# PearCoding/PearRay

Hardware: AMD Instinct MI355X
Metric: Msamples/s (higher is better)
Workload: dtype f32; 1 GPU; C4: Cornell box + 999968-triangle soup (1000000 triangles), 1920x1080, `direct` integrator (NEE+MIS+RR, depth 64), sobol 1024-spp schedule, hero wavelengths (spd CMIS), 307 iterations timed; parallelism=tiles1, collective=none (one rank)

## Files before the change

pearray_amd/csrc/device/render.h:

```cpp
#pragma once
#include "pr_device.h"

namespace prd {
constexpr int N_DEVICE_COUNTERS = PRGPU_STAT_COUNT + 32;

struct TraceWorkspace {
	uint32_t* queue_head = nullptr;
	uint2* spill		 = nullptr;
	uint32_t max_blocks	 = 0;
	int refill_below	 = 44;
	uint32_t* bl_list	 = nullptr;
	uint32_t* bl_word	 = nullptr;
	uint32_t* slot_unit	 = nullptr;
	size_t bl_entries	 = 0;
};
size_t trace_workspace_spill_entries(uint32_t max_blocks);
uint32_t trace_stack_capacity();

void launch_raygen(const DevScene& sc, const PathState& ps, uint32_t slot_base, uint32_t n_slots, uint32_t iter, unsigned long long* gstats, hipStream_t st);
void launch_trace_closest(const DevScene& sc, const PathState& ps, const uint32_t* active, uint32_t slot_base, uint32_t n_active, bool count,
						  const TraceWorkspace& ws, uint32_t* shade_counters, unsigned long long* gstats, hipStream_t st);
void launch_shade(const DevScene& sc, const PathState& ps, const uint32_t* active, uint32_t slot_base, uint32_t n_active, uint32_t* next_active,
				  uint32_t* counters, uint32_t* dead_list, uint32_t* queue_head_closest, uint32_t* queue_head_shadow, unsigned long long* gstats,
				  hipStream_t st);
void launch_regen(const DevScene& sc, const PathState& ps, const uint32_t* dead, uint32_t n_dead, uint32_t iter_end, uint32_t* next_active,
				  uint32_t* counters, unsigned long long* gstats, hipStream_t st);
void launch_trace_shadow(const DevScene& sc, const PathState& ps, uint32_t n_items, bool count, const TraceWorkspace& ws, unsigned long long* gstats,
						 hipStream_t st);
struct PersistentGeometry {
	uint32_t n_blocks, slots_per_block;
};
PersistentGeometry persistent_geometry(uint32_t n_owned, uint32_t max_blocks, uint32_t max_slots_per_block);
uint32_t persistent_slot_padding();
uint32_t slot_array_padding();
uint32_t persistent_block_threads();
int shade_ticks_counter();
struct PersistentTuning {
	uint32_t slots	  = 384;
	int shade_min	  = 64;
	int shade_partial = 16;
	int fin_batch	  = 16;
	int occupancy	  = 3;
	int shader_wave	  = -1;
	bool resident	  = true;
};
void launch_path_persistent(const DevScene& sc, const PathState& ps, const uint32_t* owned, uint32_t n_owned, uint32_t iter_begin, uint32_t iter_end,
							bool count, const TraceWorkspace& ws, const PersistentTuning& tune, int shader_waves , uint32_t* next_pixel, uint32_t* error,
							unsigned long long* gstats, hipStream_t st);
struct PathVariant {
	int id;
	uint32_t features;
};
constexpr uint32_t FEAT_NO_LPE = FEAT_ALL & ~(FEAT_LPE | FEAT_QUADRICS | FEAT_DISKS | FEAT_IMAGES | FEAT_MIX_MATERIALS | FEAT_EXPR | FEAT_SCALAR_NODES), FEAT_NO_ROUGH = FEAT_NO_LPE & ~FEAT_ROUGH_MATERIALS;
constexpr PathVariant PATH_VARIANTS[] = { { 1, 0u }, { 2, FEAT_DELTA_MATERIALS }, { 3, FEAT_NO_ROUGH }, { 4, FEAT_NO_LPE }, { 5, FEAT_ALL } };
constexpr int N_PATH_VARIANTS		  = int(sizeof(PATH_VARIANTS) / sizeof(PATH_VARIANTS[0]));
constexpr int path_variant(uint32_t features)
{
	for (int i = 0; i < N_PATH_VARIANTS - 1; ++i)
		if ((features & ~PATH_VARIANTS[i].features) == 0u)
			return i;
	return N_PATH_VARIANTS - 1;
}
constexpr int path_variant_row(int id)
{
	int i = 0;
	while (i < N_PATH_VARIANTS && PATH_VARIANTS[i].id != id)
		++i;
	return i;
}
constexpr bool path_variants_nested()
{
	for (int i = 0; i + 1 < N_PATH_VARIANTS; ++i)
		if ((PATH_VARIANTS[i].features & ~PATH_VARIANTS[i + 1].features) != 0u)
			return false;
	return true;
}
static_assert(PATH_VARIANTS[N_PATH_VARIANTS - 1].features == FEAT_ALL, "the last variant must cover every scene");
constexpr bool expr_rides_with_images()
{
	for (int i = 0; i < N_PATH_VARIANTS; ++i)
		if (((PATH_VARIANTS[i].features & FEAT_IMAGES) != 0u) != ((PATH_VARIANTS[i].features & FEAT_EXPR) != 0u))
			return false;
	return true;
}
static_assert(expr_rides_with_images(), "FEAT_EXPR and FEAT_IMAGES must sit in the same rows: the closures' _uv forms serve both");
static_assert(path_variants_nested(), "each variant's mask must be contained in the next one's: then the first covering row is the smallest covering one");
// ... 79 lines not shown
```

pearray_amd/csrc/device/render.hip:

```cpp
#define PR_WAVEFRONT 1
#define PR_THROUGHPUT 2
#define PR_LATENCY 3
#if !defined(PR_UNIT) || (PR_UNIT != PR_WAVEFRONT && PR_UNIT != PR_THROUGHPUT && PR_UNIT != PR_LATENCY)
#error "compile with -DPR_UNIT=PR_WAVEFRONT, PR_THROUGHPUT or PR_LATENCY (see the Makefile)"
#endif
#include "render.h"

#include <algorithm>
#include <array>
#include <utility>
#if PR_UNIT == PR_WAVEFRONT
#include <hipcub/hipcub.hpp>
#endif

namespace prd {

__device__ __forceinline__ unsigned long long lane_ballot(bool p) { return __builtin_amdgcn_ballot_w64(p); }
__device__ __forceinline__ bool lane_in(unsigned long long m) { return __builtin_amdgcn_inverse_ballot_w64(m); }
__device__ __forceinline__ int wave_popc(unsigned long long m)
{
	int n = __builtin_popcountll(m);
	asm volatile("" : "+s"(n));
	return n;
}

struct Hit {
	float t, u, v;
	uint32_t tri;
};

enum { CNT_NODES_CLOSEST = PRGPU_STAT_COUNT, CNT_TRIS_CLOSEST, CNT_NODES_ANY, CNT_TRIS_ANY, CNT_WAVE_ITERS_CLOSEST, CNT_WAVE_ITERS_ANY, CNT_SHADE_BATCHES, CNT_SHADE_LANES, CNT_SHADE_TICKS, CNT_IDLE_TICKS, CNT_TOTAL_TICKS, CNT_LEAF_TICKS, CNT_INNER_TICKS, CNT_TOTAL_CYCLES, CNT_REFILL_TICKS, CNT_FIN_TICKS, CNT_CAMERA_TICKS, CNT_VERTEX_TICKS,
	   CNT_CLS_TICKS0, CNT_CLS_BATCHES0 = CNT_CLS_TICKS0 + 4, CNT_CLS_LANES0 = CNT_CLS_BATCHES0 + 4,
	   CNT_SINGLES_CLOSEST = CNT_CLS_LANES0 + 4, CNT_SINGLES_ANY };

#ifndef PR_PEEK
#define PR_PEEK 0
#endif
#ifndef PR_PL_VARIANTS
#define PR_PL_VARIANTS 31
#endif
#ifndef PR_PP_BLOCK
#define PR_PP_BLOCK 256
#endif
constexpr int PP_BLOCK		= PR_PP_BLOCK;
constexpr int TRAV_BLOCK	= PR_UNIT != PR_WAVEFRONT ? PP_BLOCK : 256;
constexpr int STACK_LDS		= 16;
constexpr int STACK_SPILL	= 64;

struct Stack {
	uint2* lds;
	uint2* spill;
	uint32_t spill_stride;
	int sp, base;
	__device__ __forceinline__ void reset() { sp = base = 0; }
	__device__ __forceinline__ void reserve(int k)
	{
		while (sp - base + k > STACK_LDS) {
			if (base < STACK_SPILL)
				spill[(uint32_t)base * spill_stride] = lds[(base & (STACK_LDS - 1)) * TRAV_BLOCK];
			++base;
		}
	}
	__device__ __forceinline__ void push_if(bool valid, uint32_t ref, uint32_t key)
	{
		lds[(sp & (STACK_LDS - 1)) * TRAV_BLOCK] = make_uint2(ref, key);
		sp += valid ? 1 : 0;
	}
	__device__ __forceinline__ uint2 peek() const { return lds[((sp - 1) & (STACK_LDS - 1)) * TRAV_BLOCK]; }
	__device__ __forceinline__ uint2 pop_peeked(uint2 top)
	{
		--sp;
		if (__builtin_expect(sp < base, 0)) {
			base = sp;
			top	 = make_uint2(REC_EMPTY, 0x7F800000u);
			if (sp < STACK_SPILL)
				top = spill[(uint32_t)sp * spill_stride];
		}
		return top;
	}
	__device__ __forceinline__ uint2 pop()
	{
		--sp;
		uint2 e = lds[(sp & (STACK_LDS - 1)) * TRAV_BLOCK];
		if (__builtin_expect(sp < base, 0)) {
			base = sp;
			e	 = make_uint2(REC_EMPTY, 0x7F800000u);
// ... 2235 lines not shown
		}
	};
	trace_persistent<true, COUNT>(sc, n, queue_head, spill, refill_below, load, store, gstats);
}

__global__ void __launch_bounds__(256) k_resolve(DevScene sc, PathState ps, uint32_t iter)
{
	const uint32_t W = sc.cfg.width, H = sc.cfg.height;
	const uint32_t p = blockIdx.x * blockDim.x + threadIdx.x;
	if (p >= W * H)
		return;
	float acc[3];
	if (sc.single_tap) {
		acc[0] = ps.iter_xyz[3 * p];
		acc[1] = ps.iter_xyz[3 * p + 1];
		acc[2] = ps.iter_xyz[3 * p + 2];
	} else {
		const int r = (int)sc.cfg.filter_radius, dd = 2 * r + 1;
		const int x = (int)(p % W), y = (int)(p / W);
		acc[0] = acc[1] = acc[2] = 0.0f;
		for (int sy = y - r; sy <= y + r; ++sy) {
			if (sy < 0 || sy >= (int)H)
				continue;
			for (int sx = x - r; sx <= x + r; ++sx) {
				if (sx < 0 || sx >= (int)W)
					continue;
				const float fw = sc.filter[(y - sy + r) * dd + (x - sx + r)];
				if (fw > PR_EPS) {
					const uint32_t q = (uint32_t)sy * W + (uint32_t)sx;
					acc[0] += fw * ps.iter_xyz[3 * q];
					acc[1] += fw * ps.iter_xyz[3 * q + 1];
					acc[2] += fw * ps.iter_xyz[3 * q + 2];
				}
			}
		}
	}
	fold_iteration(ps, p, iter, acc);
}


#endif
#ifndef PR_PP_SLOTS_MAX
#define PR_PP_SLOTS_MAX (PP_BLOCK == 768 ? 1536 : 512)
#endif
#ifndef PR_FIN_PRIO
#define PR_FIN_PRIO 2
#endif
#ifndef PR_REFILL_PRIO
#define PR_REFILL_PRIO 2
#endif
#ifndef PR_SHADE_PRIO
#define PR_SHADE_PRIO 3
#endif
constexpr int PP_SLOTS_MAX		= PR_PP_SLOTS_MAX;
constexpr uint32_t WL_LDS		= 448;
constexpr uint32_t PP_EMPTY		= 0xFFFFFFFFu;
constexpr uint32_t PP_ANY		= 0x80000000u;
constexpr uint32_t PP_DEAD		= 0x100u;
constexpr uint32_t PP_VISIBLE	= 0x200u;
constexpr uint32_t PP_CLS_SHIFT	= 12u;
constexpr uint32_t PP_SHADOW	= 0x400u;
constexpr unsigned long long PP_IDLE_LIMIT_TICKS = 30ull * 100000000ull;

template <int NQ>
struct PPShared {
	uint2 stack[STACK_LDS * TRAV_BLOCK];
	uint32_t q_ray[2 * PP_SLOTS_MAX];
	uint32_t q_shade[NQ + 1][PP_SLOTS_MAX];
	uint32_t pending[PP_SLOTS_MAX];
	uint32_t ray_head, ray_tail, shade_head[NQ + 1], shade_tail[NQ + 1];
	float wl_cdf[WL_LDS];
	uint16_t wl_guide[CDF_GUIDE_BUCKETS + 2];
	uint32_t n_list, unit_next, exhausted, n_frozen;
	uint32_t live;
	uint32_t error;
	BlockStats bs;
};

__device__ __forceinline__ uint32_t lds_load(const uint32_t* p) { return __hip_atomic_load(p, __ATOMIC_RELAXED, __HIP_MEMORY_SCOPE_WORKGROUP); }
__device__ __forceinline__ uint32_t wave_bcast0(uint32_t v) { return (uint32_t)__builtin_amdgcn_readfirstlane((int)v); }

__device__ __forceinline__ void ring_push(uint32_t* q, uint32_t cap_mask, uint32_t* tail, bool pred, uint32_t value)
{
	const unsigned long long mask = __ballot(pred);
	if (mask == 0ull)
		return;
	const uint32_t lane = threadIdx.x & 63u;
	uint32_t base		= 0;
	const int leader	= __ffsll((long long)mask) - 1;
	if ((int)lane == leader)
		base = __hip_atomic_fetch_add(tail, (uint32_t)__popcll(mask), __ATOMIC_RELAXED, __HIP_MEMORY_SCOPE_WORKGROUP);
	base = __shfl(base, leader, 64);
	if (pred)
		__hip_atomic_store(&q[(base + __popcll(mask & ((1ull << lane) - 1ull))) & cap_mask], value, __ATOMIC_RELEASE, __HIP_MEMORY_SCOPE_WORKGROUP);
}
__device__ __forceinline__ uint32_t ring_claim(uint32_t* head, const uint32_t* tail, uint32_t want, uint32_t& first)
{
	uint32_t n = 0, h = 0;
	if ((threadIdx.x & 63u) == 0) {
		h				 = lds_load(head);
		const uint32_t t = lds_load(tail);
		n				 = min(want, t - h);
		if (n) {
			uint32_t expect = h;
			if (!__hip_atomic_compare_exchange_strong(head, &expect, h + n, __ATOMIC_RELAXED, __ATOMIC_RELAXED, __HIP_MEMORY_SCOPE_WORKGROUP))
				n = 0;
		}
	}
	first = wave_bcast0(h);
	return wave_bcast0(n);
}
__device__ __forceinline__ uint32_t ring_take(uint32_t* q, uint32_t cap_mask, uint32_t pos)
{
	uint32_t* e = &q[pos & cap_mask];
	uint32_t v;
	while ((v = __hip_atomic_load(e, __ATOMIC_ACQUIRE, __HIP_MEMORY_SCOPE_WORKGROUP)) == PP_EMPTY)
		__builtin_amdgcn_s_sleep(1);
	__hip_atomic_store(e, PP_EMPTY, __ATOMIC_RELAXED, __HIP_MEMORY_SCOPE_WORKGROUP);
	return v;
}


template <uint32_t FEATS>
__device__ __forceinline__ void apply_deferred_nee(const PathState& ps, uint32_t slot, uint32_t pw)
{
	if (pw & PP_SHADOW) {
		const float4 x		 = ps.st[slot].sh_xyz;
		const uint32_t fbs	 = __float_as_uint(x.w);
		const uint32_t pixel = ps.pixel[slot];
		if (pw & PP_VISIBLE) {
// ... 2 lines not shown
		} else if ((fbs >> 8) & 0xFFu) {
			ps.feedback[pixel] |= (fbs >> 8) & 0xFFu;
		}
	}
}

template <uint32_t FEATS>
__device__ __forceinline__ void fold_ended_sample(const PathState& ps, uint32_t slot, uint32_t pixel, uint32_t iter)
{
	if (ps.cost)
		ps.cost[pixel] += (ps.st[slot].flags & 0xFFu) + 1u;
	if (!ps.plane_stride) {
		const float v[3] = { ps.iter_xyz[3 * pixel], ps.iter_xyz[3 * pixel + 1], ps.iter_xyz[3 * pixel + 2] };
		fold_iteration(ps, pixel, iter, v, (FEATS & FEAT_LPE) != 0u);
	}
}


struct PersistentArgs {
	const uint32_t* owned;
	uint32_t n_owned;
	uint32_t* next_pixel;
	uint32_t* error;
	uint32_t slots_per_block;
	uint32_t iter_begin, iter_end;
	uint2* spill;
	int refill_below;
	uint32_t shade_min;
	uint32_t shade_partial;
	uint32_t shader_wave;
	int fin_batch;
	uint32_t direct_map;
	uint32_t resident;
	uint32_t bl_cap;
	uint32_t* bl_list;
	uint32_t* bl_word;
	uint32_t* slot_unit;
	unsigned long long* gstats;
};
constexpr uint32_t PP_SHADE_HELP = 128u;
constexpr uint32_t BL_UNWRITTEN = 0xFFFFFFFEu, BL_HOLE = 0xFFFFFFFFu;

template <bool COUNT, uint32_t FEATS, int WIDE>
__device__ __forceinline__ void path_persistent(const DevScene& sc, const PathState& ps, const PersistentArgs& a)
{
	constexpr int NQ = (FEATS & FEAT_ROUGH_MATERIALS) ? 2 : 1;
	constexpr int QR = NQ;
	constexpr uint32_t FEATS_PLAIN = FEATS & ~FEAT_ROUGH_MATERIALS;
	__shared__ PPShared<NQ> sh;
	constexpr uint32_t RAY_MASK = 2 * PP_SLOTS_MAX - 1, SHADE_MASK = PP_SLOTS_MAX - 1;
	const uint32_t lane	 = threadIdx.x & 63u;
	const uint32_t block_slots = a.slots_per_block;
	const uint32_t slot0	   = blockIdx.x * block_slots;
	for (uint32_t i = threadIdx.x; i < 2 * PP_SLOTS_MAX; i += TRAV_BLOCK)
		sh.q_ray[i] = PP_EMPTY;
	for (uint32_t i = threadIdx.x; i < PP_SLOTS_MAX; i += TRAV_BLOCK) {
		sh.q_shade[QR][i] = i < block_slots ? i : PP_EMPTY;
		for (int q = 0; q < NQ; ++q)
			sh.q_shade[q][i] = PP_EMPTY;
		sh.pending[i] = 0;
		if (i < block_slots)
			ps.pixel[slot0 + i] = INVALID;
	}
	if (threadIdx.x == 0) {
		sh.ray_head = sh.ray_tail = 0;
		for (int q = 0; q < NQ; ++q)
			sh.shade_head[q] = sh.shade_tail[q] = 0;
		sh.shade_head[QR] = 0;
		sh.shade_tail[QR] = block_slots;
		sh.live					  = block_slots;
		sh.error				  = 0;
		sh.n_list = sh.unit_next = sh.exhausted = sh.n_frozen = 0;
	}
	uint32_t* const bl_list = a.bl_list + size_t(blockIdx.x) * a.bl_cap;
	uint32_t* const bl_word = a.bl_word + size_t(blockIdx.x) * a.bl_cap;
	if (a.resident)
		for (uint32_t i = threadIdx.x; i < a.bl_cap; i += TRAV_BLOCK) {
			bl_list[i] = BL_UNWRITTEN;
			bl_word[i] = 0u;
		}
	const bool wl_in_lds = sc.wl_cdf_size >= 2u && sc.wl_cdf_size <= WL_LDS && sc.cfg.mapper == PRGPU_MAPPER_SPD_CMIS;
	if (wl_in_lds)
		for (uint32_t i = threadIdx.x; i < sc.wl_cdf_size; i += TRAV_BLOCK)
			sh.wl_cdf[i] = sc.wl_cdf[i];
	stats_init(sh.bs);
	__syncthreads();
	if (wl_in_lds) {
		for (uint32_t b = threadIdx.x; b <= CDF_GUIDE_BUCKETS; b += TRAV_BLOCK) {
			const float x = (float)b / (float)CDF_GUIDE_BUCKETS;
			int first = 0, len = (int)sc.wl_cdf_size;
			while (len > 0) {
				const int half = len / 2, middle = first + half;
				if (sh.wl_cdf[middle] <= x) {
					first = middle + 1;
					len -= half + 1;
				} else {
					len = half;
				}
			}
			sh.wl_guide[b] = (uint16_t)first;
		}
		__syncthreads();
	}
	WlTable wlt;
	if (wl_in_lds) {
		wlt.cdf	  = sh.wl_cdf;
		wlt.guide = sh.wl_guide;
	}

	Stack st;
	Trav s;
	trav_attach(s, st, sh.stack, a.spill);
	s.any			  = false;
	bool has_ray	  = false;
	uint32_t my_entry = 0;

	uint32_t spins	  = 0;
	unsigned long long t_idle_since = 0;
	uint32_t cn_c = 0, cl_c = 0, cn_a = 0, cl_a = 0, cs_c = 0, cs_a = 0, witers = 0, wleaf = 0, sbatches = 0, slanes = 0;
	unsigned long long t_shade = 0, t_idle = 0, t_leaf = 0, t_inner = 0, t_refill = 0, t_fin = 0, t_cam = 0, t_vert = 0;
	unsigned long long t_cls[4] = { 0, 0, 0, 0 };
	uint32_t b_cls[4] = { 0, 0, 0, 0 }, l_cls[4] = { 0, 0, 0, 0 };
	const unsigned long long t_start = COUNT ? wall_clock64() : 0ull;
	const unsigned long long c_start = COUNT ? (unsigned long long)clock64() : 0ull;

	const uint32_t shader_idx = 3u;
	const bool shader		  = a.shader_wave != 0u && ((threadIdx.x >> 6) & 3u) + a.shader_wave > shader_idx;
	const uint32_t shade_full = a.shader_wave != 0u ? PP_SHADE_HELP : a.shade_min;
	for (;;) {
		const int n_act	  = __popcll(__ballot(has_ray));
		uint32_t n_shade = wave_bcast0(lds_load(&sh.shade_tail[0]) - lds_load(&sh.shade_head[0]));
		int cls			 = 0;
		for (int q = 1; q < NQ + 1; ++q) {
			const uint32_t nq = wave_bcast0(lds_load(&sh.shade_tail[q]) - lds_load(&sh.shade_head[q]));
			if (nq > n_shade) {
				n_shade = nq;
				cls		= q;
			}
		}
		uint32_t n_queued = wave_bcast0(lds_load(&sh.ray_tail) - lds_load(&sh.ray_head));

		bool shade_now;
		if (shader)
			shade_now = n_shade > 0u;
		else if (a.shader_wave != 0u)
			shade_now = n_shade >= shade_full || (n_queued == 0u && n_shade > 0u && n_act == 0);
		else
			shade_now = n_shade >= a.shade_min || (n_queued == 0u && ((n_shade >= a.shade_partial && n_act < a.refill_below) || (n_shade > 0u && n_act == 0)));
		if (shade_now) {
			uint32_t first;
			const uint32_t n = ring_claim(&sh.shade_head[cls], &sh.shade_tail[cls], 64u, first);
			if (n) {
				spins			  = 0;
#if PR_SHADE_PRIO
				__builtin_amdgcn_s_setprio(PR_SHADE_PRIO);
#endif
				const unsigned long long t0 = COUNT ? wall_clock64() : 0ull;
				if (COUNT && lane == 0) {
					++sbatches;
					slanes += n;
				}
				const bool mine	  = lane < n;
				uint32_t slot_l	  = 0;
				const bool regen_pass = cls == QR;
				const bool regen	  = regen_pass;
				if (mine)
					slot_l = ring_take(sh.q_shade[cls], SHADE_MASK, first + lane);
				const uint32_t slot = slot0 + slot_l;
				if (mine)
					apply_deferred_nee<FEATS>(ps, slot, lds_load(&sh.pending[slot_l]));
				bool alive = false, want_shadow = false;
				float4 sh_o = make_float4(0, 0, 0, 0), sh_d = sh_o, sh_xyz = sh_o;
				const unsigned long long t0v = COUNT ? wall_clock64() : 0ull;
				if (regen_pass) {
				} else if (NQ > 1 && cls == 1) {
					if (mine)
						shade_vertex<FEATS>(sc, ps, slot, sh.bs, alive, want_shadow, sh_o, sh_d, sh_xyz);
				} else {
					if (mine)
						shade_vertex<FEATS_PLAIN>(sc, ps, slot, sh.bs, alive, want_shadow, sh_o, sh_d, sh_xyz);
				}
				if (COUNT)
					t_vert += wall_clock64() - t0v;
				const bool to_regen = !regen_pass && mine && !alive && !want_shadow;
				const bool ended	= mine && regen;
				bool need_pixel	 = false;
				uint32_t iter	 = 0;
				if (ended) {
					const uint32_t pixel = ps.pixel[slot];
					need_pixel			 = true;
					if (pixel != INVALID) {
						iter = ps.iter[slot];
						fold_ended_sample<FEATS>(ps, slot, pixel, iter);
						if (iter + 1 < a.iter_end) {
							if (!a.resident) {
								need_pixel = false;
								iter	   = iter + 1;
							} else {
								const uint32_t old = __hip_atomic_fetch_add(&bl_word[a.slot_unit[slot]], 1u, __ATOMIC_ACQ_REL, __HIP_MEMORY_SCOPE_WORKGROUP);
								if ((old >> 16) >= (old & 0xFFFFu) + 1u) {
									need_pixel = false;
									iter	   = iter + 1;
								}
							}
						}
					}
				}
				bool retired = false;
				if (a.resident) {
					if (wave_bcast0(lds_load(&sh.exhausted)) == 0u) {
						const unsigned long long m = __ballot(need_pixel);
						if (m != 0ull) {
							const uint32_t n	= (uint32_t)__popcll(m);
							const uint32_t rank = (uint32_t)__popcll(m & ((1ull << lane) - 1ull));
							const int leader	= __ffsll((long long)m) - 1;
							uint32_t pos		= 0;
							if ((int)lane == leader)
								pos = __hip_atomic_fetch_add(&sh.n_list, n, __ATOMIC_RELAXED, __HIP_MEMORY_SCOPE_WORKGROUP);
							pos = __shfl(pos, leader, 64);
							const uint32_t n_fit = pos >= a.bl_cap ? 0u : min(n, a.bl_cap - pos);
							uint32_t idx		 = a.n_owned;
							if (n_fit != 0u) {
								__builtin_amdgcn_fence(__ATOMIC_SEQ_CST, "workgroup");
								if ((int)lane == leader)
									idx = atomicAdd(a.next_pixel, n_fit);
								idx = __shfl(idx, leader, 64);
							}
							if ((n_fit < n || idx + n_fit >= a.n_owned) && (int)lane == leader)
								__hip_atomic_store(&sh.exhausted, 1u, __ATOMIC_RELEASE, __HIP_MEMORY_SCOPE_WORKGROUP);
							if (need_pixel && rank < n_fit) {
								const uint32_t i = idx + rank;
								uint32_t entry	 = BL_HOLE;
								if (i < a.n_owned) {
// ... 62 lines not shown
							iter		   = a.iter_begin;
						} else {
							retired = true;
						}
					}
				}
				const unsigned long long t0c = COUNT ? wall_clock64() : 0ull;
				if (ended && !retired) {
					ps.iter[slot] = iter;
					camera_path(sc, ps, slot, iter, sh.bs, (FEATS & FEAT_LPE) != 0u, wlt);
					alive = true;
				}
				if (COUNT)
					t_cam += wall_clock64() - t0c;
				const int n_retired = __popcll(__ballot(retired));
				if (n_retired && lane == 0)
					__hip_atomic_fetch_sub(&sh.live, (uint32_t)n_retired, __ATOMIC_RELAXED, __HIP_MEMORY_SCOPE_WORKGROUP);
				if (mine && !retired) {
					if (want_shadow) {
						ps.st[slot].sh_o	= sh_o;
						ps.st[slot].sh_d	= sh_d;
						ps.st[slot].sh_xyz = sh_xyz;
					}
					__hip_atomic_store(&sh.pending[slot_l], (alive ? 1u : 0u) + (want_shadow ? 1u + PP_SHADOW : 0u) + (alive ? 0u : PP_DEAD), __ATOMIC_RELAXED,
									   __HIP_MEMORY_SCOPE_WORKGROUP);
				}
				ring_push(sh.q_shade[QR], SHADE_MASK, &sh.shade_tail[QR], to_regen, slot_l);
				ring_push(sh.q_ray, RAY_MASK, &sh.ray_tail, want_shadow, slot_l | PP_ANY);
				ring_push(sh.q_ray, RAY_MASK, &sh.ray_tail, alive, slot_l);
				{
					const uint32_t pslot = slot0 + (has_ray ? (my_entry & ~PP_ANY) : 0u);
					const bool pany		 = has_ray && (my_entry & PP_ANY) != 0;
					const float4 ro = pany ? ps.st[pslot].sh_o : ps.st[pslot].ray_o, rd = pany ? ps.st[pslot].sh_d : ps.st[pslot].ray_d;
					s.r	   = ray_prepare(v3(ro.x, ro.y, ro.z), v3(rd.x, rd.y, rd.z), sc.eps_t);
					s.tmin = ro.w + 0.0f;
					s.any  = pany;
				}
#if PR_SHADE_PRIO
				__builtin_amdgcn_s_setprio(0);
#endif
				if (COUNT)
					t_shade += wall_clock64() - t0;
				if (COUNT && lane == 0)
					for (int q = 0; q < NQ + 1; ++q)
						if (q == cls) {
							t_cls[q] += wall_clock64() - t0;
							b_cls[q] += 1u;
							l_cls[q] += n;
						}
			}
			continue;
		}

		const unsigned long long idle = __ballot(!has_ray);
		if (!shader && idle != 0ull && n_queued > 0u) {
#if PR_REFILL_PRIO
			__builtin_amdgcn_s_setprio(PR_REFILL_PRIO);
#endif
			const unsigned long long t0r = COUNT ? wall_clock64() : 0ull;
			uint32_t first;
			const uint32_t n = ring_claim(&sh.ray_head, &sh.ray_tail, (uint32_t)__popcll(idle), first);
			const uint32_t r = __popcll(idle & ((1ull << lane) - 1ull));
			if (!has_ray && r < n) {
				my_entry			= ring_take(sh.q_ray, RAY_MASK, first + r);
				const uint32_t slot = slot0 + (my_entry & ~PP_ANY);
				const bool any		= (my_entry & PP_ANY) != 0;
				const float4 ro = any ? ps.st[slot].sh_o : ps.st[slot].ray_o, rd = any ? ps.st[slot].sh_d : ps.st[slot].ray_d;
				trav_begin(s, st, v3(ro.x, ro.y, ro.z), v3(rd.x, rd.y, rd.z), ro.w, any ? rd.w - 0.001f : rd.w, sc.eps_t);
				s.any	= any;
				has_ray = true;
				if (FEATS & FEAT_QUADRICS)
					trav_quadrics<(NQ > 1)>(sc, s, any);
			}
#if PR_REFILL_PRIO
			__builtin_amdgcn_s_setprio(0);
#endif
			if (COUNT)
				t_refill += wall_clock64() - t0r;
		}
		if (!__any(has_ray)) {
			if (lds_load(&sh.live) == 0u || lds_load(&sh.error) != 0u)
				break;
			const unsigned long long t0 = COUNT ? wall_clock64() : 0ull;
			__builtin_amdgcn_s_sleep(8);
			if (COUNT)
				t_idle += wall_clock64() - t0;
			if (n_shade == 0u && n_queued == 0u) {
				if (spins++ == 0u)
					t_idle_since = wall_clock64();
				else if ((spins & 1023u) == 0u && wall_clock64() - t_idle_since > PP_IDLE_LIMIT_TICKS) {
					if (lane == 0) {
						__hip_atomic_store(&sh.error, 1u, __ATOMIC_RELAXED, __HIP_MEMORY_SCOPE_WORKGROUP);
						atomicExch(a.error, 1u);
					}
					break;
				}
			}
			continue;
		}
		spins = 0;
		unsigned long long m_has  = lane_ballot(has_ray);
		unsigned long long m_wait = m_has & lane_ballot(s.cur == REC_EMPTY);
		for (;;) {
			const unsigned long long m_lb	 = lane_ballot((s.cur & REC_LEAF_BIT) != 0u);
			const unsigned long long m_leaf	 = m_has & m_lb & ~m_wait;
			const unsigned long long m_inner = m_has & ~m_lb;
			const int n_leaf = wave_popc(m_leaf), n_inner = wave_popc(m_inner);
			if (COUNT && lane == 0)
				++witers;
			const bool do_inner = n_inner >= n_leaf;
			const unsigned long long t0s = COUNT ? wall_clock64() : 0ull;
			if (lane_in(do_inner ? m_inner : m_leaf)) {
				const float4* __restrict__ rec = rec_ptr(sc.recs, s.cur);
				const float4 q0 = rec[0], q1 = rec[1], q2 = rec[2];
				const bool wide = WIDE == 2 ? sc.bvh_wide != 0u : WIDE == 1;
				float4 qw		= make_float4(0.0f, 0.0f, 0.0f, 0.0f);
				if (wide && do_inner)
					qw = rec[3];
				const uint2 top_e	   = PR_PEEK ? st.peek() : make_uint2(0u, 0u);
				const uint2* const top = PR_PEEK ? &top_e : nullptr;
				if (do_inner) {
					if (COUNT) {
						cn_c += s.any ? 0 : 1;
						cn_a += s.any ? 1 : 0;
					}
					trav_inner_rec<MODE_MIXED>(s, st, q0, q1, q2, qw, wide, top);
				} else {
					float4 q3 = make_float4(0.0f, 0.0f, 0.0f, 0.0f), q4 = q3, q5 = q3, q6 = q3, q7 = q3;
					if (!(s.cur & REC_SINGLE_BIT)) {
						q3 = rec[3];
						q4 = rec[4];
						q5 = rec[5];
						q6 = rec[6];
						q7 = rec[7];
					}
					if (COUNT) {
						cl_c += s.any ? 0 : 1;
						cl_a += s.any ? 1 : 0;
						if (s.cur & REC_SINGLE_BIT) {
							cs_c += s.any ? 0 : 1;
							cs_a += s.any ? 1 : 0;
						}
					}
					trav_leaf_rec<MODE_MIXED, (FEATS & ANA_ALL), (NQ > 1)>(s, st, q0, q1, q2, q3, q4, q5, q6, q7, top);
				}
			}
			if (COUNT) {
				if (do_inner)
					t_inner += wall_clock64() - t0s;
				else
					t_leaf += wall_clock64() - t0s;
			}
			const unsigned long long m_done = m_has & lane_ballot(s.cur == REC_EMPTY);
			unsigned long long m_fin		= m_done;
			if (a.fin_batch > 1) {
				const int n_done = wave_popc(m_done);
				const int n_run	 = wave_popc(m_has & ~m_done);
				if (n_done < a.fin_batch && n_run >= a.refill_below)
					m_fin = 0ull;
			}
			const unsigned long long t0f = COUNT ? wall_clock64() : 0ull;
			if (m_fin != 0ull) {
#if PR_FIN_PRIO
				__builtin_amdgcn_s_setprio(PR_FIN_PRIO);
#endif
				const bool fin = lane_in(m_fin);
				bool last	   = false;
				uint32_t entry = 0;
				int qcls	   = 0;
				if (fin) {
					const uint32_t slot_l = my_entry & ~PP_ANY;
					const uint32_t slot	  = slot0 + slot_l;
					uint32_t add = 0xFFFFFFFFu;
					if (s.any) {
						if (s.best.tri == INVALID)
							add += PP_VISIBLE;
					} else {
						ps.st[slot].hit = make_float4(s.best.t, s.best.u, s.best.v, __uint_as_float(s.best.tri));
						if (NQ > 1)
							add += (s.cls & 3u) << PP_CLS_SHIFT;
					}
					const uint32_t old = __hip_atomic_fetch_add(&sh.pending[slot_l], add, __ATOMIC_ACQ_REL, __HIP_MEMORY_SCOPE_WORKGROUP);
					last			   = (old & 0xFFu) == 1u;
					entry			   = slot_l;
					if (last && (old & PP_DEAD))
						qcls = QR;
					if (NQ > 1 && last && !(old & PP_DEAD))
						qcls = s.any ? (int)((old >> PP_CLS_SHIFT) & 3u) : (int)(s.cls & 3u);
				}
				m_has &= ~m_fin;
				for (int q = 0; q < NQ + 1; ++q)
					ring_push(sh.q_shade[q], SHADE_MASK, &sh.shade_tail[q], last && qcls == q, entry);
#if PR_FIN_PRIO
				__builtin_amdgcn_s_setprio(0);
#endif
				if (COUNT)
					t_fin += wall_clock64() - t0f;
			}
			m_wait			 = m_done & m_has;
			const int active = wave_popc(m_has);
			if (active == 0)
				break;
			if (active < a.refill_below) {
				uint32_t nsh = lds_load(&sh.shade_tail[0]) - lds_load(&sh.shade_head[0]);
				for (int q = 1; q < NQ + 1; ++q)
					nsh = max(nsh, lds_load(&sh.shade_tail[q]) - lds_load(&sh.shade_head[q]));
				const uint32_t nq = lds_load(&sh.ray_tail) - lds_load(&sh.ray_head);
				if (wave_bcast0((nq > 0u || nsh >= shade_full || (a.shader_wave == 0u && nsh >= a.shade_partial)) ? 1u : 0u))
					break;
			}
		}
		has_ray = lane_in(m_has);
	}
	if (COUNT) {
		if (cn_c)
			atomicAdd(&a.gstats[CNT_NODES_CLOSEST], (unsigned long long)cn_c);
		if (cl_c)
			atomicAdd(&a.gstats[CNT_TRIS_CLOSEST], (unsigned long long)cl_c);
		if (cn_a)
			atomicAdd(&a.gstats[CNT_NODES_ANY], (unsigned long long)cn_a);
		if (cl_a)
			atomicAdd(&a.gstats[CNT_TRIS_ANY], (unsigned long long)cl_a);
		if (cs_c)
			atomicAdd(&a.gstats[CNT_SINGLES_CLOSEST], (unsigned long long)cs_c);
		if (cs_a)
			atomicAdd(&a.gstats[CNT_SINGLES_ANY], (unsigned long long)cs_a);
		if (witers)
			atomicAdd(&a.gstats[CNT_WAVE_ITERS_CLOSEST], (unsigned long long)witers);
		if (wleaf)
			atomicAdd(&a.gstats[CNT_WAVE_ITERS_ANY], (unsigned long long)wleaf);
		if (sbatches) {
			atomicAdd(&a.gstats[CNT_SHADE_BATCHES], (unsigned long long)sbatches);
			atomicAdd(&a.gstats[CNT_SHADE_LANES], (unsigned long long)slanes);
		}
		if (lane == 0) {
			atomicAdd(&a.gstats[CNT_SHADE_TICKS], t_shade);
			atomicAdd(&a.gstats[CNT_IDLE_TICKS], t_idle);
			atomicAdd(&a.gstats[CNT_TOTAL_TICKS], wall_clock64() - t_start);
			atomicAdd(&a.gstats[CNT_LEAF_TICKS], t_leaf);
			atomicAdd(&a.gstats[CNT_INNER_TICKS], t_inner);
			atomicAdd(&a.gstats[CNT_REFILL_TICKS], t_refill);
			atomicAdd(&a.gstats[CNT_FIN_TICKS], t_fin);
			atomicAdd(&a.gstats[CNT_CAMERA_TICKS], t_cam);
			atomicAdd(&a.gstats[CNT_VERTEX_TICKS], t_vert);
			atomicAdd(&a.gstats[CNT_TOTAL_CYCLES], (unsigned long long)clock64() - c_start);
			for (int q = 0; q < NQ + 1; ++q) {
				atomicAdd(&a.gstats[CNT_CLS_TICKS0 + q], t_cls[q]);
				atomicAdd(&a.gstats[CNT_CLS_BATCHES0 + q], (unsigned long long)b_cls[q]);
				atomicAdd(&a.gstats[CNT_CLS_LANES0 + q], (unsigned long long)l_cls[q]);
			}
		}
		if (threadIdx.x == 0)
			a.spill[blockIdx.x * TRAV_BLOCK] = make_uint2((uint32_t)(wall_clock64() - t_start), sh.bs.v[PRGPU_STAT_CAMERA_DEPTH] + sh.bs.v[PRGPU_STAT_BACKGROUND_HITS]);
	}
	stats_flush(sh.bs, a.gstats);
}
template <bool COUNT, uint32_t FEATS>
__global__ void __launch_bounds__(TRAV_BLOCK) __attribute__((amdgpu_waves_per_eu(2, 2))) k_path_persistent(DevScene sc, PathState ps, PersistentArgs a)
{
	path_persistent<COUNT, FEATS, 2>(sc, ps, a);
}
template <bool COUNT, uint32_t FEATS, bool WIDE>
__global__ void __launch_bounds__(TRAV_BLOCK) __attribute__((amdgpu_waves_per_eu(3, 3))) k_path_persistent_occ3(DevScene sc, PathState ps, PersistentArgs a)
{
	path_persistent<COUNT, FEATS, WIDE ? 1 : 0>(sc, ps, a);
}

#include "path_wave.inl"

#if PR_UNIT == PR_WAVEFRONT
struct CameraVertex {
	uint32_t pixel;
	float4 hit4;
	V3 ray_d, P;
	GeomPoint gp;
};
enum { CV_NONE, CV_BACKGROUND, CV_HIT };
__device__ __forceinline__ int camera_vertex(const DevScene& sc, const PathState& ps, uint32_t slot, uint32_t n_slots, BlockStats& bs, CameraVertex& cv)
{
	if (slot >= n_slots || (ps.st[slot].flags & FLAG_NO_RAY))
		return CV_NONE;
	const uint32_t pixel = ps.pixel[slot];
	const float4 hit4	 = ps.st[slot].hit;
	const uint32_t tri	 = __float_as_uint(hit4.w);
	cv.pixel			 = pixel;
	cv.hit4				 = hit4;
	if (tri == INVALID) {
		ps.prim_entity[pixel] = INVALID;
		ps.prim_prim[pixel]	  = INVALID;
		atomicAdd(&bs.v[PRGPU_STAT_BACKGROUND_HITS], 1u);
		return CV_BACKGROUND;
	}
	const float4 ro = ps.st[slot].ray_o, rd = ps.st[slot].ray_d;
	const V3 ray_o = v3(ro.x, ro.y, ro.z), ray_d = v3(rd.x, rd.y, rd.z);
	const V3 P = ray_o + ray_d * hit4.x;
	geometry_point<(FEAT_ALL & ~FEAT_LPE)>(sc, tri, hit4.y, hit4.z, P, cv.gp);
	ps.prim_entity[pixel] = cv.gp.entity;
	ps.prim_prim[pixel]	  = cv.gp.prim;
// ... 438 lines not shown
}
bool ao_counts_folded() { return PR_AO_FOLD != 0; }
void launch_vf_shade(const DevScene& sc, const PathState& ps, const VfState& vf, uint32_t n_slots, uint32_t* queue_head_closest, unsigned long long* gstats, hipStream_t st)
{
	hipLaunchKernelGGL(k_vf_shade, grid_for(n_slots), dim3(256), 0, st, sc, ps, vf, n_slots, queue_head_closest, gstats);
}

#endif

template <int VARIANT, int SUB>
void launch_pp(const DevScene& sc, const PathState& ps, const PersistentArgs& a, dim3 grid, hipStream_t st);
template <int VARIANT, int SUB>
void launch_pl(const DevScene& sc, const PathState& ps, const WaveArgs& a, dim3 grid, hipStream_t st);
#if PR_UNIT != PR_WAVEFRONT
#if !defined(PR_VARIANT) || !defined(PR_SUB)
#error "compile the persistent-kernel units with -DPR_VARIANT=<id of a row of PATH_VARIANTS> -DPR_SUB=<index>"
#endif
static_assert(path_variant_row(PR_VARIANT) < N_PATH_VARIANTS, "PR_VARIANT is not the id of a row of PATH_VARIANTS");
#if PR_UNIT == PR_LATENCY
template <int VARIANT, int SUB>
void launch_pl(const DevScene& sc, const PathState& ps, const WaveArgs& a, dim3 grid, hipStream_t st)
{
	static_assert(SUB == 0 || SUB == 1, "latency units: PR_SUB=0 (plain) or 1 (instrumented)");
	hipLaunchKernelGGL((k_path_latency<SUB != 0, PATH_VARIANTS[path_variant_row(VARIANT)].features>), grid, dim3(TRAV_BLOCK), 0, st, sc, ps, a);
}
template void launch_pl<PR_VARIANT, PR_SUB>(const DevScene&, const PathState&, const WaveArgs&, dim3, hipStream_t);
#else
template <int VARIANT, int SUB>
void launch_pp(const DevScene& sc, const PathState& ps, const PersistentArgs& a, dim3 grid, hipStream_t st)
{
	constexpr PathSub u		 = PATH_SUBS[SUB];
	constexpr uint32_t FEATS = PATH_VARIANTS[path_variant_row(VARIANT)].features;
	const dim3 block(TRAV_BLOCK);
	if constexpr (u.occupancy == 3)
		hipLaunchKernelGGL((k_path_persistent_occ3<u.count, FEATS, u.wide>), grid, block, 0, st, sc, ps, a);
	else
		hipLaunchKernelGGL((k_path_persistent<u.count, FEATS>), grid, block, 0, st, sc, ps, a);
}
template void launch_pp<PR_VARIANT, PR_SUB>(const DevScene&, const PathState&, const PersistentArgs&, dim3, hipStream_t);
#endif
#endif

#if PR_UNIT == PR_WAVEFRONT
PersistentGeometry persistent_geometry(uint32_t n_owned, uint32_t max_blocks, uint32_t max_slots_per_block)
{
	PersistentGeometry g;
	const uint32_t per_block = (n_owned + max_blocks - 1) / std::max(1u, max_blocks);
	const uint32_t cap		 = std::min((uint32_t)PP_SLOTS_MAX, std::max(256u, max_slots_per_block / 64u * 64u));
	g.slots_per_block		 = std::min(cap, std::max(64u, per_block));
	g.n_blocks				 = std::max(1u, std::min(max_blocks, (n_owned + g.slots_per_block - 1) / g.slots_per_block));
	return g;
}
uint32_t persistent_slot_padding() { return PP_SLOTS_MAX; }
uint32_t slot_array_padding() { return std::max<uint32_t>(PP_SLOTS_MAX, (TRAV_BLOCK / 64u) * PW_SLOTS_MAX); }
uint32_t persistent_block_threads() { return PP_BLOCK; }
int shade_ticks_counter() { return CNT_SHADE_TICKS; }

typedef void (*PpLaunchFn)(const DevScene&, const PathState&, const PersistentArgs&, dim3, hipStream_t);
typedef void (*PlLaunchFn)(const DevScene&, const PathState&, const WaveArgs&, dim3, hipStream_t);
template <int... I>
constexpr std::array<PpLaunchFn, sizeof...(I)> pp_launch_table(std::integer_sequence<int, I...>)
{
	return { { launch_pp<PATH_VARIANTS[I / N_PATH_SUBS].id, I % N_PATH_SUBS>... } };
}
constexpr bool pl_variant_built(int row) { return ((PR_PL_VARIANTS >> (PATH_VARIANTS[row].id - 1)) & 1u) != 0u; }
template <int ROW, int SUB>
constexpr PlLaunchFn pl_launcher()
{
	if constexpr (pl_variant_built(ROW))
		return launch_pl<PATH_VARIANTS[ROW].id, SUB>;
	else
		return nullptr;
}
template <int... I>
constexpr std::array<PlLaunchFn, sizeof...(I)> pl_launch_table(std::integer_sequence<int, I...>)
{
	return { { pl_launcher<I / 2, I % 2>()... } };
}

void launch_path_persistent(const DevScene& sc, const PathState& ps, const uint32_t* owned, uint32_t n_owned, uint32_t iter_begin, uint32_t iter_end,
							bool count, const TraceWorkspace& ws, const PersistentTuning& tune, int shader_waves, uint32_t* next_pixel, uint32_t* error,
							unsigned long long* gstats, hipStream_t st)
{
	const uint32_t max_slots_per_block = tune.slots;
	const PersistentGeometry g = persistent_geometry(n_owned, ws.max_blocks, max_slots_per_block);
	const bool all_in_flight   = uint64_t(g.n_blocks) * g.slots_per_block >= n_owned;
	PersistentArgs a;
	a.owned			  = owned;
	a.n_owned		  = n_owned;
	a.next_pixel	  = next_pixel;
	a.error			  = error;
	a.slots_per_block = g.slots_per_block;
	a.iter_begin	  = iter_begin;
	a.iter_end		  = iter_end;
	a.spill			  = ws.spill;
	a.refill_below	  = ws.refill_below;
	a.shade_min		  = (uint32_t)std::min(64, std::max(1, tune.shade_min));
	a.shade_partial	  = (uint32_t)std::min(64, std::max(1, tune.shade_partial));
	a.shader_wave	  = PP_BLOCK == 256 ? (uint32_t)std::min(2, std::max(0, shader_waves)) : (shader_waves ? 1u : 0u);
	a.gstats		  = gstats;
	a.direct_map	  = all_in_flight ? 1u : 0u;
	a.fin_batch		  = std::min(64, std::max(1, tune.fin_batch));
	const bool resident_ok = tune.resident;
	a.bl_cap		  = (uint32_t)std::min<uint64_t>(n_owned, 2ull * ((n_owned + g.n_blocks - 1) / g.n_blocks) + 1024ull);
	a.bl_list		  = ws.bl_list;
	a.bl_word		  = ws.bl_word;
// ... 60 lines not shown
```

pearray_amd/csrc/prgpu_api.hip:

```cpp
#include <hip/hip_runtime.h>
#include <dlfcn.h>

#include <algorithm>
#include <climits>
#include <cmath>
#include <cstdlib>
#include <cstring>
#include <map>
#include <string>
#include <vector>

#include "../../include/prgpu.h"
#include "device/bvh.h"
#include "device/render.h"
#include "host/mix_tree.h"
#include "host/setup.h"
#include "tables/pr_vf_colors.inl"
static_assert(sizeof(PR_VF_COLOR_RGB) / sizeof(PR_VF_COLOR_RGB[0]) == prd::VF_COLOURS, "one row per colour index of device/render.h");

namespace {

thread_local std::string g_error;

int fail(int code, const std::string& msg)
// ... 1456 lines not shown

int prgpu_film_size(prgpu_scene* s, uint32_t* width, uint32_t* height)
{
	if (!s)
		return fail(PRGPU_EINVAL, "null scene");
	if (width)
		*width = s->cfg.width;
	if (height)
		*height = s->cfg.height;
	return PRGPU_OK;
}

int prgpu_trace_counters_get(prgpu_scene* s, prgpu_trace_counters* out)
{
	if (!s || !out)
		return fail(PRGPU_EINVAL, "null argument");
	HIP_TRY(hipSetDevice(s->device));
	HIP_TRY(hipStreamSynchronize(s->stream));
	unsigned long long host[prd::N_DEVICE_COUNTERS];
	HIP_TRY(hipMemcpy(host, s->gstats, sizeof(host), hipMemcpyDeviceToHost));
	out->rays_closest  = s->rays_closest;
	out->rays_any	   = s->rays_any;
	if (s->mode == prgpu_scene::PERSISTENT || s->ao_enabled || s->vf_enabled) {
		out->rays_closest += host[PRGPU_STAT_PRIMARY_RAYS] + host[PRGPU_STAT_BOUNCE_RAYS];
		out->rays_any += host[PRGPU_STAT_SHADOW_RAYS];
	}
	out->nodes_closest = host[PRGPU_STAT_COUNT + 0];
	out->leaves_closest  = host[PRGPU_STAT_COUNT + 1];
	out->nodes_any	   = host[PRGPU_STAT_COUNT + 2];
	out->leaves_any	   = host[PRGPU_STAT_COUNT + 3];
	out->node_bytes	   = sizeof(prd::Rec64);
	out->leaf_bytes	   = 2 * sizeof(prd::Rec64);
	if (s->bvh_leaf == 1) {
		out->leaf_bytes		= sizeof(prd::Rec64);
		out->leaves_closest = 2 * out->leaves_closest - host[PRGPU_STAT_COUNT + 30];
		out->leaves_any		= 2 * out->leaves_any - host[PRGPU_STAT_COUNT + 31];
	}
	out->ray_bytes	   = 32;
	out->hit_bytes	   = 16;
	out->wave_steps_closest = host[PRGPU_STAT_COUNT + 4];
	out->wave_steps_any		= host[PRGPU_STAT_COUNT + 5];
	out->shade_batches		= host[PRGPU_STAT_COUNT + 6];
	out->shade_lanes		= host[PRGPU_STAT_COUNT + 7];
	out->shade_ticks		= host[PRGPU_STAT_COUNT + 8];
	out->idle_ticks			= host[PRGPU_STAT_COUNT + 9];
	out->total_ticks		= host[PRGPU_STAT_COUNT + 10];
	if (read_knobs().debug_counters)
		if (host[PRGPU_STAT_COUNT + 10]) {
			const double T = double(host[PRGPU_STAT_COUNT + 10]);
			fprintf(stderr, "[prgpu] wave time: shading %.1f %%, idle %.1f %%, leaf steps %.1f %%, inner steps %.1f %%, refill %.1f %%, ray ends %.1f %%; of the shading: vertices %.1f %%, camera paths %.1f %%; shader clock %.0f MHz\n",
					100 * host[PRGPU_STAT_COUNT + 8] / T, 100 * host[PRGPU_STAT_COUNT + 9] / T, 100 * host[PRGPU_STAT_COUNT + 11] / T, 100 * host[PRGPU_STAT_COUNT + 12] / T,
					100 * host[PRGPU_STAT_COUNT + 14] / T, 100 * host[PRGPU_STAT_COUNT + 15] / T, 100 * host[PRGPU_STAT_COUNT + 17] / T, 100 * host[PRGPU_STAT_COUNT + 16] / T,
					100.0 * double(host[PRGPU_STAT_COUNT + 13]) / T);
			for (int q = 0; q < 4; ++q)
				if (host[PRGPU_STAT_COUNT + 22 + q])
					fprintf(stderr, "[prgpu]   shade queue %d: %.1f %% of wave time, %.0f passes, fill %.3f, %.2f us per pass\n", q, 100 * host[PRGPU_STAT_COUNT + 18 + q] / T,
							double(host[PRGPU_STAT_COUNT + 22 + q]), double(host[PRGPU_STAT_COUNT + 26 + q]) / (64.0 * double(host[PRGPU_STAT_COUNT + 22 + q])),
							0.01 * double(host[PRGPU_STAT_COUNT + 18 + q]) / double(host[PRGPU_STAT_COUNT + 22 + q]));
		}
	return PRGPU_OK;
}

int prgpu_set_instrumentation(prgpu_scene* s, int enabled)
{
	if (!s)
		return fail(PRGPU_EINVAL, "null scene");
	s->instrument = enabled != 0;
	return PRGPU_OK;
}

int prgpu_set_timing(prgpu_scene* s, int enabled)
{
	if (!s)
		return fail(PRGPU_EINVAL, "null scene");
	HIP_TRY(hipSetDevice(s->device));
	HIP_TRY(hipStreamSynchronize(s->stream));
	s->collect_timing();
	s->timing = enabled != 0;
	return PRGPU_OK;
}

int prgpu_kernel_time_ms(prgpu_scene* s, const char* family, double* total_ms, uint64_t* launches)
{
	if (!s || !family)
		return fail(PRGPU_EINVAL, "null argument");
	HIP_TRY(hipSetDevice(s->device));
	HIP_TRY(hipStreamSynchronize(s->stream));
	s->collect_timing();
	for (int f = 0; f < N_FAMILIES; ++f)
		if (std::strcmp(family, FAMILY_NAMES[f]) == 0) {
			if (total_ms)
				*total_ms = s->family_ms[f];
			if (launches)
				*launches = s->family_launches[f];
			return PRGPU_OK;
		}
	return fail(PRGPU_EINVAL, "unknown kernel family");
}

int prgpu_trace_closest(prgpu_scene* s, uint32_t n, const float* org, const float* dir, const float* tmin, const float* tmax,
						uint32_t* entity, uint32_t* prim, float* u, float* v, float* t)
{
	if (!s || (n && (!org || !dir || !tmin || !tmax)))
		return fail(PRGPU_EINVAL, "null argument");
	if (n == 0)
		return PRGPU_OK;
// ... 679 lines not shown
```

Measured before the change: 224.9 Msamples/s.

## Overlap ray pickup with traversal steps and keep hit records in LDS

Splits the refill of idle lanes into an issue phase (claiming queue entries and loading ray origin and direction from global slot records) and a finish phase (traversal setup) that runs after the next traversal step. This lets the global loads overlap with BVH stepping instead of breaking out of the inner loop whenever rays are queued. Closest-hit results are also kept in a per-block LDS array and passed to shade_vertex, avoiding a global store and reload when the block's slot count fits. The LDS footprint grows, and static_asserts check that three 256-lane blocks still fit per CU. New lane-step counters and a debug print are added.

New measurement: 222.5 Msamples/s. 1.1% lower.

```diff
diff --git a/pearray_amd/csrc/device/render.h b/pearray_amd/csrc/device/render.h
--- a/pearray_amd/csrc/device/render.h
+++ b/pearray_amd/csrc/device/render.h
@@ -2,7 +2,7 @@
 #include "pr_device.h"
 
 namespace prd {
-constexpr int N_DEVICE_COUNTERS = PRGPU_STAT_COUNT + 32;
+constexpr int N_DEVICE_COUNTERS = PRGPU_STAT_COUNT + 36;
 
 struct TraceWorkspace {
 	uint32_t* queue_head = nullptr;
@@ -32,6 +32,7 @@
 };
 PersistentGeometry persistent_geometry(uint32_t n_owned, uint32_t max_blocks, uint32_t max_slots_per_block);
 uint32_t persistent_slot_padding();
+uint32_t persistent_hit_slots(uint32_t features);
 uint32_t slot_array_padding();
 uint32_t persistent_block_threads();
 int shade_ticks_counter();
diff --git a/pearray_amd/csrc/device/render.hip b/pearray_amd/csrc/device/render.hip
--- a/pearray_amd/csrc/device/render.hip
+++ b/pearray_amd/csrc/device/render.hip
@@ -31,7 +31,8 @@
 
 enum { CNT_NODES_CLOSEST = PRGPU_STAT_COUNT, CNT_TRIS_CLOSEST, CNT_NODES_ANY, CNT_TRIS_ANY, CNT_WAVE_ITERS_CLOSEST, CNT_WAVE_ITERS_ANY, CNT_SHADE_BATCHES, CNT_SHADE_LANES, CNT_SHADE_TICKS, CNT_IDLE_TICKS, CNT_TOTAL_TICKS, CNT_LEAF_TICKS, CNT_INNER_TICKS, CNT_TOTAL_CYCLES, CNT_REFILL_TICKS, CNT_FIN_TICKS, CNT_CAMERA_TICKS, CNT_VERTEX_TICKS,
 	   CNT_CLS_TICKS0, CNT_CLS_BATCHES0 = CNT_CLS_TICKS0 + 4, CNT_CLS_LANES0 = CNT_CLS_BATCHES0 + 4,
-	   CNT_SINGLES_CLOSEST = CNT_CLS_LANES0 + 4, CNT_SINGLES_ANY };
+	   CNT_SINGLES_CLOSEST = CNT_CLS_LANES0 + 4, CNT_SINGLES_ANY,
+	   CNT_LANES_STEPPED, CNT_LANES_OTHER, CNT_LANES_WAITING, CNT_LANES_EMPTY, CNT_END };
 
 #ifndef PR_PEEK
 #define PR_PEEK 0
@@ -2373,7 +2374,14 @@
 #ifndef PR_SHADE_PRIO
 #define PR_SHADE_PRIO 3
 #endif
+#ifndef PR_PP_PICKUP
+#define PR_PP_PICKUP 1
+#endif
+#ifndef PR_PP_HIT_LDS
+#define PR_PP_HIT_LDS 1
+#endif
 constexpr int PP_SLOTS_MAX		= PR_PP_SLOTS_MAX;
+constexpr uint32_t pp_hit_slots(int nq) { return PR_PP_HIT_LDS ? (nq > 1 ? uint32_t(PP_SLOTS_MAX) * 3u / 4u : uint32_t(PP_SLOTS_MAX)) : 1u; }
 constexpr uint32_t WL_LDS		= 448;
 constexpr uint32_t PP_EMPTY		= 0xFFFFFFFFu;
 constexpr uint32_t PP_ANY		= 0x80000000u;
@@ -2389,6 +2397,7 @@
 	uint32_t q_ray[2 * PP_SLOTS_MAX];
 	uint32_t q_shade[NQ + 1][PP_SLOTS_MAX];
 	uint32_t pending[PP_SLOTS_MAX];
+	float4 hit[pp_hit_slots(NQ)];
 	uint32_t ray_head, ray_tail, shade_head[NQ + 1], shade_tail[NQ + 1];
 	float wl_cdf[WL_LDS];
 	uint16_t wl_guide[CDF_GUIDE_BUCKETS + 2];
@@ -2397,6 +2406,11 @@
 	uint32_t error;
 	BlockStats bs;
 };
+static_assert(CNT_END == N_DEVICE_COUNTERS, "render.h: N_DEVICE_COUNTERS must hold every counter");
+constexpr size_t LDS_UNIT = 1280, LDS_UNITS_PER_CU = 128;
+static_assert(PP_BLOCK != 256 || 3 * ((sizeof(PPShared<2>) + LDS_UNIT - 1) / LDS_UNIT) <= LDS_UNITS_PER_CU, "three blocks of 256 lanes must fit a CU's LDS");
+static_assert(PP_BLOCK != 256 || 3 * ((sizeof(PPShared<1>) + LDS_UNIT - 1) / LDS_UNIT) <= LDS_UNITS_PER_CU, "three blocks of 256 lanes must fit a CU's LDS");
+static_assert(sizeof(PPShared<2>) <= LDS_UNIT * LDS_UNITS_PER_CU, "a block must fit a CU's LDS");
 
 __device__ __forceinline__ uint32_t lds_load(const uint32_t* p) { return __hip_atomic_load(p, __ATOMIC_RELAXED, __HIP_MEMORY_SCOPE_WORKGROUP); }
 __device__ __forceinline__ uint32_t wave_bcast0(uint32_t v) { return (uint32_t)__builtin_amdgcn_readfirstlane((int)v); }
@@ -2505,6 +2519,7 @@
 	const uint32_t lane	 = threadIdx.x & 63u;
 	const uint32_t block_slots = a.slots_per_block;
 	const uint32_t slot0	   = blockIdx.x * block_slots;
+	const bool hit_lds = PR_PP_HIT_LDS && block_slots <= pp_hit_slots(NQ);
 	for (uint32_t i = threadIdx.x; i < 2 * PP_SLOTS_MAX; i += TRAV_BLOCK)
 		sh.q_ray[i] = PP_EMPTY;
 	for (uint32_t i = threadIdx.x; i < PP_SLOTS_MAX; i += TRAV_BLOCK) {
@@ -2574,11 +2589,12 @@
 	unsigned long long t_shade = 0, t_idle = 0, t_leaf = 0, t_inner = 0, t_refill = 0, t_fin = 0, t_cam = 0, t_vert = 0;
 	unsigned long long t_cls[4] = { 0, 0, 0, 0 };
 	uint32_t b_cls[4] = { 0, 0, 0, 0 }, l_cls[4] = { 0, 0, 0, 0 };
+	unsigned long long ls_step = 0, ls_other = 0, ls_wait = 0, ls_empty = 0;
 	const unsigned long long t_start = COUNT ? wall_clock64() : 0ull;
 	const unsigned long long c_start = COUNT ? (unsigned long long)clock64() : 0ull;
 
 	const uint32_t shader_idx = 3u;
-	const bool shader		  = a.shader_wave != 0u && ((threadIdx.x >> 6) & 3u) + a.shader_wave > shader_idx;
+	const bool shader		  = wave_bcast0((a.shader_wave != 0u && ((threadIdx.x >> 6) & 3u) + a.shader_wave > shader_idx) ? 1u : 0u) != 0u;
 	const uint32_t shade_full = a.shader_wave != 0u ? PP_SHADE_HELP : a.shade_min;
 	for (;;) {
 		const int n_act	  = __popcll(__ballot(has_ray));
@@ -2625,13 +2641,20 @@
 				bool alive = false, want_shadow = false;
 				float4 sh_o = make_float4(0, 0, 0, 0), sh_d = sh_o, sh_xyz = sh_o;
 				const unsigned long long t0v = COUNT ? wall_clock64() : 0ull;
+				float4 hit4 = make_float4(0.0f, 0.0f, 0.0f, 0.0f);
+				if (!regen_pass && mine) {
+					if (hit_lds)
+						hit4 = sh.hit[slot_l];
+					else
+						hit4 = ps.st[slot].hit;
+				}
 				if (regen_pass) {
 				} else if (NQ > 1 && cls == 1) {
 					if (mine)
-						shade_vertex<FEATS>(sc, ps, slot, sh.bs, alive, want_shadow, sh_o, sh_d, sh_xyz);
+						shade_vertex<FEATS>(sc, ps, slot, sh.bs, alive, want_shadow, sh_o, sh_d, sh_xyz, &hit4);
 				} else {
 					if (mine)
-						shade_vertex<FEATS_PLAIN>(sc, ps, slot, sh.bs, alive, want_shadow, sh_o, sh_d, sh_xyz);
+						shade_vertex<FEATS_PLAIN>(sc, ps, slot, sh.bs, alive, want_shadow, sh_o, sh_d, sh_xyz, &hit4);
 				}
 				if (COUNT)
 					t_vert += wall_clock64() - t0v;
@@ -2800,33 +2823,52 @@
 			continue;
 		}
 
+		auto pickup_issue = [&](unsigned long long m_idle) -> unsigned long long {
+			uint32_t first;
+			const uint32_t n = ring_claim(&sh.ray_head, &sh.ray_tail, (uint32_t)wave_popc(m_idle), first);
+			const uint32_t r = __popcll(m_idle & ((1ull << lane) - 1ull));
+			const bool take	 = lane_in(m_idle) && r < n;
+			if (take) {
+				my_entry			= ring_take(sh.q_ray, RAY_MASK, first + r);
+				const uint32_t slot = slot0 + (my_entry & ~PP_ANY);
+				const bool any		= (my_entry & PP_ANY) != 0;
+				const float4 ro = any ? ps.st[slot].sh_o : ps.st[slot].ray_o, rd = any ? ps.st[slot].sh_d : ps.st[slot].ray_d;
+				s.r.o	 = v3(ro.x, ro.y, ro.z);
+				s.r.d	 = v3(rd.x, rd.y, rd.z);
+				s.tmin	 = ro.w;
+				s.best.t = rd.w;
+			}
+			return lane_ballot(take);
+		};
+		auto pickup_finish = [&](unsigned long long m_arriving) {
+			if (lane_in(m_arriving)) {
+				const bool any = (my_entry & PP_ANY) != 0;
+				trav_begin(s, st, s.r.o, s.r.d, s.tmin, any ? s.best.t - 0.001f : s.best.t, sc.eps_t);
+				s.any = any;
+				if (FEATS & FEAT_QUADRICS)
+					trav_quadrics<(NQ > 1)>(sc, s, any);
+			}
+		};
+		unsigned long long m_arr	  = 0ull;
 		const unsigned long long idle = __ballot(!has_ray);
 		if (!shader && idle != 0ull && n_queued > 0u) {
 #if PR_REFILL_PRIO
 			__builtin_amdgcn_s_setprio(PR_REFILL_PRIO);
 #endif
 			const unsigned long long t0r = COUNT ? wall_clock64() : 0ull;
-			uint32_t first;
-			const uint32_t n = ring_claim(&sh.ray_head, &sh.ray_tail, (uint32_t)__popcll(idle), first);
-			const uint32_t r = __popcll(idle & ((1ull << lane) - 1ull));
-			if (!has_ray && r < n) {
-				my_entry			= ring_take(sh.q_ray, RAY_MASK, first + r);
-				const uint32_t slot = slot0 + (my_entry & ~PP_ANY);
-				const bool any		= (my_entry & PP_ANY) != 0;
-				const float4 ro = any ? ps.st[slot].sh_o : ps.st[slot].ray_o, rd = any ? ps.st[slot].sh_d : ps.st[slot].ray_d;
-				trav_begin(s, st, v3(ro.x, ro.y, ro.z), v3(rd.x, rd.y, rd.z), ro.w, any ? rd.w - 0.001f : rd.w, sc.eps_t);
-				s.any	= any;
-				has_ray = true;
-				if (FEATS & FEAT_QUADRICS)
-					trav_quadrics<(NQ > 1)>(sc, s, any);
-			}
+			m_arr						 = pickup_issue(idle);
+#if !PR_PP_PICKUP
+			pickup_finish(m_arr);
+			has_ray = has_ray || lane_in(m_arr);
+			m_arr	= 0ull;
+#endif
 #if PR_REFILL_PRIO
 			__builtin_amdgcn_s_setprio(0);
 #endif
 			if (COUNT)
 				t_refill += wall_clock64() - t0r;
 		}
-		if (!__any(has_ray)) {
+		if (!__any(has_ray) && m_arr == 0ull) {
 			if (lds_load(&sh.live) == 0u || lds_load(&sh.error) != 0u)
 				break;
 			const unsigned long long t0 = COUNT ? wall_clock64() : 0ull;
@@ -2857,6 +2899,12 @@
 			if (COUNT && lane == 0)
 				++witers;
 			const bool do_inner = n_inner >= n_leaf;
+			if (COUNT) {
+				ls_step += (unsigned long long)(do_inner ? n_inner : n_leaf);
+				ls_other += (unsigned long long)(do_inner ? n_leaf : n_inner);
+				ls_wait += (unsigned long long)wave_popc(m_wait);
+				ls_empty += (unsigned long long)(64 - wave_popc(m_has));
+			}
 			const unsigned long long t0s = COUNT ? wall_clock64() : 0ull;
 			if (lane_in(do_inner ? m_inner : m_leaf)) {
 				const float4* __restrict__ rec = rec_ptr(sc.recs, s.cur);
@@ -2899,6 +2947,14 @@
 				else
 					t_leaf += wall_clock64() - t0s;
 			}
+			if (m_arr != 0ull) {
+				const unsigned long long t0r = COUNT ? wall_clock64() : 0ull;
+				pickup_finish(m_arr);
+				m_has |= m_arr;
+				m_arr = 0ull;
+				if (COUNT)
+					t_refill += wall_clock64() - t0r;
+			}
 			const unsigned long long m_done = m_has & lane_ballot(s.cur == REC_EMPTY);
 			unsigned long long m_fin		= m_done;
 			if (a.fin_batch > 1) {
@@ -2924,7 +2980,11 @@
 						if (s.best.tri == INVALID)
 							add += PP_VISIBLE;
 					} else {
-						ps.st[slot].hit = make_float4(s.best.t, s.best.u, s.best.v, __uint_as_float(s.best.tri));
+						const float4 h = make_float4(s.best.t, s.best.u, s.best.v, __uint_as_float(s.best.tri));
+						if (hit_lds)
+							sh.hit[slot_l] = h;
+						else
+							ps.st[slot].hit = h;
 						if (NQ > 1)
 							add += (s.cls & 3u) << PP_CLS_SHIFT;
 					}
@@ -2954,8 +3014,20 @@
 				for (int q = 1; q < NQ + 1; ++q)
 					nsh = max(nsh, lds_load(&sh.shade_tail[q]) - lds_load(&sh.shade_head[q]));
 				const uint32_t nq = lds_load(&sh.ray_tail) - lds_load(&sh.ray_head);
+#if PR_PP_PICKUP
+				const uint32_t todo = wave_bcast0((nsh >= shade_full || (nq == 0u && a.shader_wave == 0u && nsh >= a.shade_partial)) ? 2u : (nq > 0u ? 1u : 0u));
+				if (todo == 2u)
+					break;
+				if (todo == 1u) {
+					const unsigned long long t0r = COUNT ? wall_clock64() : 0ull;
+					m_arr						 = pickup_issue(~m_has);
+					if (COUNT)
+						t_refill += wall_clock64() - t0r;
+				}
+#else
 				if (wave_bcast0((nq > 0u || nsh >= shade_full || (a.shader_wave == 0u && nsh >= a.shade_partial)) ? 1u : 0u))
 					break;
+#endif
 			}
 		}
 		has_ray = lane_in(m_has);
@@ -2992,6 +3064,10 @@
 			atomicAdd(&a.gstats[CNT_CAMERA_TICKS], t_cam);
 			atomicAdd(&a.gstats[CNT_VERTEX_TICKS], t_vert);
 			atomicAdd(&a.gstats[CNT_TOTAL_CYCLES], (unsigned long long)clock64() - c_start);
+			atomicAdd(&a.gstats[CNT_LANES_STEPPED], ls_step);
+			atomicAdd(&a.gstats[CNT_LANES_OTHER], ls_other);
+			atomicAdd(&a.gstats[CNT_LANES_WAITING], ls_wait);
+			atomicAdd(&a.gstats[CNT_LANES_EMPTY], ls_empty);
 			for (int q = 0; q < NQ + 1; ++q) {
 				atomicAdd(&a.gstats[CNT_CLS_TICKS0 + q], t_cls[q]);
 				atomicAdd(&a.gstats[CNT_CLS_BATCHES0 + q], (unsigned long long)b_cls[q]);
@@ -3536,6 +3612,7 @@
 	return g;
 }
 uint32_t persistent_slot_padding() { return PP_SLOTS_MAX; }
+uint32_t persistent_hit_slots(uint32_t features) { return pp_hit_slots((PATH_VARIANTS[path_variant(features)].features & FEAT_ROUGH_MATERIALS) ? 2 : 1); }
 uint32_t slot_array_padding() { return std::max<uint32_t>(PP_SLOTS_MAX, (TRAV_BLOCK / 64u) * PW_SLOTS_MAX); }
 uint32_t persistent_block_threads() { return PP_BLOCK; }
 int shade_ticks_counter() { return CNT_SHADE_TICKS; }
diff --git a/pearray_amd/csrc/prgpu_api.hip b/pearray_amd/csrc/prgpu_api.hip
--- a/pearray_amd/csrc/prgpu_api.hip
+++ b/pearray_amd/csrc/prgpu_api.hip
@@ -1532,6 +1532,11 @@
 					100 * host[PRGPU_STAT_COUNT + 8] / T, 100 * host[PRGPU_STAT_COUNT + 9] / T, 100 * host[PRGPU_STAT_COUNT + 11] / T, 100 * host[PRGPU_STAT_COUNT + 12] / T,
 					100 * host[PRGPU_STAT_COUNT + 14] / T, 100 * host[PRGPU_STAT_COUNT + 15] / T, 100 * host[PRGPU_STAT_COUNT + 17] / T, 100 * host[PRGPU_STAT_COUNT + 16] / T,
 					100.0 * double(host[PRGPU_STAT_COUNT + 13]) / T);
+			const double L = double(host[PRGPU_STAT_COUNT + 32]) + double(host[PRGPU_STAT_COUNT + 33]) + double(host[PRGPU_STAT_COUNT + 34]) + double(host[PRGPU_STAT_COUNT + 35]);
+			if (L > 0.0 && s->pp_last_kernel == PRGPU_KERNEL_THROUGHPUT)
+				fprintf(stderr, "[prgpu] lane steps: stepped %.4f, other record kind %.4f, finished and waiting %.4f, no ray %.4f; hits travel through %s (%u slots per block, LDS holds the hits of %u)\n",
+						host[PRGPU_STAT_COUNT + 32] / L, host[PRGPU_STAT_COUNT + 33] / L, host[PRGPU_STAT_COUNT + 34] / L, host[PRGPU_STAT_COUNT + 35] / L,
+						s->pp_last_slots <= prd::persistent_hit_slots(s->sc.features) ? "LDS" : "the slot record", s->pp_last_slots, prd::persistent_hit_slots(s->sc.features));
 			for (int q = 0; q < 4; ++q)
 				if (host[PRGPU_STAT_COUNT + 22 + q])
 					fprintf(stderr, "[prgpu]   shade queue %d: %.1f %% of wave time, %.0f passes, fill %.3f, %.2f us per pass\n", q, 100 * host[PRGPU_STAT_COUNT + 18 + q] / T,
```
